# Lymphatus/caesium-clt

Hardware: AMD Instinct MI355X
Metric: megapixels/sec JPEG q=80 1920x1080 batch (higher is better)
Workload: dtype int32

## Files before the change

### caesium-clt_amd/csrc/batch.hpp

```cpp
#pragma once
#include <array>
#include <chrono>
#include <map>
#include <string>
#include <vector>

#include "../../include/caesium_hip.h"
#include "devmem.hpp"
#include "jpeg_host.hpp"
#include "kernels.h"
#include "webp_kernels.h"

namespace csh {

struct Item {
    int code = 0;
    std::string msg;
    JpegInfo in;
    JpegInfo out;
    int image = -1;
    size_t file_size = 0;
    std::vector<uint8_t> meta_out;
};

// ... 41 lines not shown
    uint32_t max_src_px = 0;
    uint64_t plane_bytes = 0, oplane_bytes = 0;
    uint32_t max_quads = 0;
    bool any_layout = false, any_layout_rgb = false;

    DevBuf<uint8_t> d_planes, d_oplanes, d_rgb;
    DevBuf<PlaneWork> d_pwork;
    DevBuf<ResizeWork> d_rwork;
    DevBuf<ResizeTap> d_rtaps;
    DevBuf<float> d_rweights, d_rtmp;
    DevBuf<int16_t> d_dct_raw;
};

struct Stage {
    uint32_t work0 = 0, nwork = 0, slot0 = 0, nslots = 0, ech0 = 0, nech = 0, table0 = 0, ntables = 0, plan0 = 0, nplans = 0, nzc0 = 0, nnzc = 0, ls0 = 0, nls = 0, ts0 = 0, nts = 0, rs0 = 0, nrs = 0, lr0 = 0, nlr = 0, rr0 = 0, nrr = 0;
    bool nz_build[2] = {true, true}, nz_filter[2] = {true, true};
};
struct SearchImg {
    int cand_work[64]; int ncand;
    int Al_luma = 0, Al_chroma = 0;
    uint64_t best_luma = 0, best_chroma = 0;
    int split_luma = 0, split_chroma = 0;
    bool luma_on = false, chroma_on = false;
};

struct EncodePlan {
    std::vector<EncScan> script;
    std::vector<ScanWork> swork;
    uint32_t nslots = 0, nlist_slots = 0, ntok_slots = 0;
    uint32_t nref_slots = 0;
    uint32_t last_run_refine = 0;
    uint32_t list_run = CSH_LIST_RUN;
    uint32_t nlist_runs = 0, nref_runs = 0;
    uint32_t last_run_list_runs = 0;
    uint64_t total_corr = 0;
    uint64_t total_units = 0, total_words = 0;
    uint32_t max_units = 0;
    int ntables = 0;
    std::vector<TokPlan> plans;
    std::vector<int> plan_comp, plan_image;
    std::vector<EChunk> echunks;
    uint64_t tok_cap = 0;
    uint32_t tok_scale = 1;
    std::vector<TokRegion> regions;
    std::vector<uint32_t> region_est;
    uint32_t hist_rows = 0;
    std::vector<NzList> nzlists;
    std::vector<NzSet> nzsets;
    std::vector<int> nzset_of;
    std::vector<uint32_t> nzset_built;
    std::vector<int> nzset_comp, nzset_image;
    std::vector<NzChunk> nzchunks;
    std::vector<NzChunk> nzchunks_fused;
    uint32_t n_fused = 0;
    uint32_t last_run_fused = 0;
    uint32_t n_ac_lists = 0;
    uint32_t last_run_ac_lists = 0;
    std::vector<uint8_t> nzset_ac_lists;
    std::vector<uint32_t> nz_est, nz_worst;
    uint32_t nz_nrec = 0;
    uint64_t nz_cap = 0;
    bool search = false;
    enum { ST_1 = 0, ST_1B = 1, ST_2 = 2, ST_2B = 3, ST_2C = 4, ST_N = 5 };
    Stage stage[ST_N];
    void stage_begin(Stage &sg) {
        sg.work0 = uint32_t(swork.size()); sg.slot0 = nslots; sg.ech0 = uint32_t(echunks.size()); sg.table0 = uint32_t(ntables); sg.plan0 = uint32_t(plans.size());
// ... 116 lines not shown
    KS_FF_COUNT, KS_SCAN_SEARCH, KS_LAYOUT, KS_SCAN_IMAGES, KS_EMIT, KS_SPARE0, KS_SPARE1, KS_SPARE2, KS_COUNT,
    KS_WEBP_YUV = KS_XFORM_DIRECT, KS_WEBP_ENCODE = KS_RESAMPLE_FDCT, KS_WEBP_ASSEMBLE = KS_FIX_DUMMY
};
struct KernelSlotRow { KernelSlot slot; const char *name; int phase; };
constexpr KernelSlotRow kKernelSlots[] = {
    {KS_MEMSET_COEF, "memset_coef", 0},        {KS_UNSTUFF, "unstuff", 0},                 {KS_DEC_SPEC, "k_dec_spec", 0},
    {KS_DEC_RELAX0, "k_dec_relax0", 0},        {KS_DEC_RELAX, "k_dec_relax1_4", 0},        {KS_DEC_WRITE, "k_dec_write", 0},
    {KS_DC_SCATTER, "k_dc_scatter", 0},        {KS_REFINE_CHAINS, "k_refine_chains", 0},   {KS_DECODE_PROG_SEQ, "k_decode_prog+seq", 0},
    {KS_IDCT_PLANE, "k_idct_plane", 1},        {KS_RESIZE, "resize", 1},                   {KS_XFORM_DIRECT, "k_xform_direct", 1},
    {KS_RESAMPLE_FDCT, "k_resample+k_plane_fdct", 1}, {KS_FIX_DUMMY, "k_fix_dummy", 1},    {KS_MEMSET_ENC, "memset_enc", 2},
    {KS_TRELLIS_STATS, "trellis_stats", 1},    {KS_TRELLIS_AC, "k_trellis_ac", 1},         {KS_TRELLIS_DC, "k_trellis_dc", 1},
    {KS_NZLIST, "k_nzlist", 2},                {KS_TOKENS, "k_tokens", 2},                 {KS_LIST_STATS, "k_list_stats", 2},
    {KS_AC_RUNS, "k_ac_runs", 2},              {KS_GEN_TABLES, "k_gen_tables", 3},         {KS_CHUNK_SIZES, "k_chunk_sizes", 4},
    {KS_SCAN_CHUNK_BITS, "scan_chunk_bits", 4}, {KS_SCAN_LAYOUT, "scan_layout", 4},        {KS_PACK, "k_pack", 5},
    {KS_LIST_PACK, "k_list_pack", 5},          {KS_FF_COUNT, "k_ff_count", 6},             {KS_SCAN_SEARCH, "scan_search_stage2", 7},
    {KS_LAYOUT, "k_layout", 6},                {KS_SCAN_IMAGES, "scan_images", 6},         {KS_EMIT, "k_emit", 6},
    {KS_SPARE0, "", 7},                        {KS_SPARE1, "", 7},                         {KS_SPARE2, "", 7}};
constexpr bool kernel_slots_in_order() {
    for (int i = 0; i < int(sizeof kKernelSlots / sizeof kKernelSlots[0]); i++) if (kKernelSlots[i].slot != i) return false;
    return true;
}
static_assert(sizeof kKernelSlots / sizeof kKernelSlots[0] == CSH_NKERNELS && int(KS_COUNT) == int(CSH_NKERNELS), "one row per csh_timing.kernel_ms slot");
static_assert(kernel_slots_in_order(), "row i of kKernelSlots describes slot i");

struct PlanSwitches {
    std::string profile;
    bool nz_once = true;
    bool tr_sort = true;
    int prog_par = -1;
    bool fused_420 = true;
    bool nz_fused = true;
    bool ref_list = true;
    uint32_t list_run = CSH_LIST_RUN;
    bool ac_tiles = false;
    static PlanSwitches read();
};

struct Laps {
    const bool trace;
    std::chrono::steady_clock::time_point at = std::chrono::steady_clock::now();
    std::string text;
    Laps();
    void lap(const char *what);
};

struct BatchPlanner {
    csh_batch *const b;
    const CByteArray *const inputs;
    const size_t count;
    const CCSParameters *const p;
    const csp_pixels *const px;
    const PlanSwitches sw;
    const bool progressive;
    uint16_t qout_nat[64];
    int script_base3 = 0, script_base1 = 0;
    std::vector<std::pair<std::vector<uint8_t>, int>> hset_keys;
    std::map<std::vector<uint16_t>, int> quant_index;
    uint64_t plane_off = 64, oplane_off = 0;

    BatchPlanner(csh_batch *b, const CByteArray *inputs, size_t count, const CCSParameters *p, const csp_pixels *px);
    void begin();
    void parse();
    int reserve_pinned();
    int plan_image(size_t n);
    int plan_search_stages();
    int plan_trellis();
// ... 35 lines not shown
```

### caesium-clt_amd/csrc/batch_plan.cpp

```cpp
#include <algorithm>
#include <atomic>
#include <cmath>
#include <thread>

#include "batch.hpp"
#include "resize_host.h"

namespace csh {

static void build_dev_huff(const HuffSpec &h, DevHuff &d) {
    memset(&d, 0, sizeof d);
    for (int l = 0; l < 18; l++) d.maxcode[l] = -1;
    if (!h.present) return;
    int code = 0, p = 0;
    for (int l = 1; l <= 16; l++) {
        if (h.bits[l]) {
            d.valptr[l] = p - code;
            for (int i = 0; i < h.bits[l]; i++, p++, code++)
                if (l <= 9) {
                    int base = code << (9 - l);
                    for (int k = 0; k < (1 << (9 - l)); k++) d.look[(base + k) & 511] = uint16_t((l << 8) | h.vals[p]);
                }
            d.maxcode[l] = code - 1;
        }
// ... 166 lines not shown
    b->enc.regions.resize(b->enc.region_est.size());
    if (b->test_pool_shift < 0) b->test_pool_shift = getenv("CSH_TEST_POOL_SHIFT") ? std::min(16, std::max(0, atoi(getenv("CSH_TEST_POOL_SHIFT")))) : 0;
    const int shift = b->test_pool_shift;
    uint64_t at = 0;
    for (size_t i = 0; i < b->enc.regions.size(); i++) {
        const uint64_t cap = std::min<uint64_t>(std::max<uint64_t>((uint64_t(b->enc.region_est[i]) * b->enc.tok_scale) >> shift, 64), 0xFFFFFFF0ull);
        b->enc.regions[i].base = at; b->enc.regions[i].cap = uint32_t(cap); b->enc.regions[i].pad = 0;
        at += (cap + 3) & ~uint64_t(3);
    }
    b->enc.tok_cap = at + 64;
    at = 0;
    for (size_t i = 0; i < b->enc.nzlists.size(); i++) {
        const uint64_t cap = std::min<uint64_t>(std::max<uint64_t>((uint64_t(b->enc.nz_est[i]) * b->enc.tok_scale) >> shift, 64), b->enc.nz_worst[i]);
        b->enc.nzlists[i].base = at; b->enc.nzlists[i].cap = uint32_t(cap);
        at += (cap + 3) & ~uint64_t(3);
    }
    b->enc.nz_cap = at + 64;
}

PlanSwitches PlanSwitches::read() {
    auto is = [](const char *name, const char *v) { const char *e = getenv(name); return e && !strcmp(e, v); };
    PlanSwitches s;
    const char *penv = getenv("CSH_PROFILE");
    s.profile = penv && *penv ? penv : "mozjpeg";
    s.nz_once = !is("CSH_NZ_ONCE", "0");
    s.tr_sort = !is("CSH_TR_SORT", "0");
    s.nz_fused = !is("CSH_NZ_FUSED", "0");
    s.ac_tiles = is("CSH_AC_TILES", "1");
    s.ref_list = is("CSH_REF_LIST", "1") || (s.ref_list && !is("CSH_REF_LIST", "0"));
    const char *pp = getenv("CSH_PROG_PAR");
    s.prog_par = pp && !strcmp(pp, "0") ? 0 : (pp && !strcmp(pp, "1") ? 1 : -1);
    s.fused_420 = !getenv("CSH_NO_FUSED_420");
    if (const char *lr = getenv("CSH_LIST_RUN")) { if (*lr) s.list_run = uint32_t(std::min(32, std::max(1, atoi(lr)))); }
    return s;
}

Laps::Laps() : trace(getenv("CSH_TRACE") != nullptr) {}
void Laps::lap(const char *what) {
    if (!trace) return;
    const auto now = std::chrono::steady_clock::now();
    char buf[64];
    snprintf(buf, sizeof buf, " %s %.1f", what, std::chrono::duration<double, std::milli>(now - at).count());
    text += buf; at = now;
}

BatchPlanner::BatchPlanner(csh_batch *b_, const CByteArray *inputs_, size_t count_, const CCSParameters *p_, const csp_pixels *px_)
    : b(b_), inputs(inputs_), count(count_), p(p_), px(px_), sw(PlanSwitches::read()), progressive(p_->jpeg_progressive) {}

void BatchPlanner::begin() {
    b->items.resize(count);
    quality_table(int(p->jpeg_quality), qout_nat);
    DevQuant qo; make_quant(qout_nat, qo);
    b->quants.push_back(qo);
    b->q_base = int(b->quants.size()) - 1;
    for (int q = 1; q <= 100; q++) { uint16_t tq[64]; quality_table(q, tq); DevQuant dq; make_quant(tq, dq); b->quants.push_back(dq); }
    b->progressive = progressive;
    b->enc.list_run = sw.list_run;

    add_script(b->enc.script, 3, true);
    add_script(b->enc.script, 1, true);
    add_script(b->enc.script, 3, false);
    add_script(b->enc.script, 1, false);
    script_base3 = progressive ? 0 : 16; script_base1 = progressive ? 10 : 17;
    const bool webp = b->webp, rgb_out = b->rgb_out;
    const std::string &profile = sw.profile;
    b->enc.search = progressive && !webp && !rgb_out && profile != "plain";
    const bool lossy_jpeg = !b->lossless && !webp && !rgb_out;
    b->tr.trellis = lossy_jpeg && (profile == "mozjpeg" || profile == "mozjpeg-trellis");
    b->tr.dering = lossy_jpeg && (profile == "mozjpeg" || profile == "mozjpeg-dering");
    b->tr.nz_once = b->tr.trellis && progressive && sw.nz_once && sw.tr_sort;
}

template <class Fill>
int BatchPlanner::enc_scan(const std::array<int, 5> &key, Fill fill) {
    auto f = b->enc.cand_script.find(key);
    if (f != b->enc.cand_script.end()) return f->second;
    EncScan e;
    memset(&e, 0, sizeof e);
    fill(e);
    b->enc.script.push_back(e);
    return b->enc.cand_script[key] = int(b->enc.script.size()) - 1;
}
int BatchPlanner::cand_index(int comp, int Ss, int Se, int Ah, int Al) {
    return enc_scan({comp, Ss, Se, Ah, Al}, [&](EncScan &e) {
        const int id = comp ? 1 : 0;
        e.ncomp = 1; e.comp[0] = comp; e.Ss = Ss; e.Se = Se; e.Ah = Ah; e.Al = Al;
        e.ntables = 1; e.dht_id[0] = 0x10 | id; e.sos_tdta[0] = id;
    });
}
int BatchPlanner::dc_scan_index(int ncomp) {
// ... 824 lines not shown
```

### caesium-clt_amd/csrc/batch_run.cpp

```cpp
#include <algorithm>

#include "batch.hpp"

namespace csh {
namespace {

class KernelMarks {
    hipEvent_t ev[CSH_NKERNELS + 1];
    int created = 0, next = 0;
    const hipStream_t st;

public:
    explicit KernelMarks(hipStream_t s) : st(s) {}
    KernelMarks(const KernelMarks &) = delete;
    KernelMarks &operator=(const KernelMarks &) = delete;
    ~KernelMarks() { for (int i = 0; i < created; i++) (void)hipEventDestroy(ev[i]); }
    int start() {
        for (; created <= CSH_NKERNELS; created++) CSH_CHECK(hipEventCreate(&ev[created]));
        CSH_CHECK(hipEventRecord(ev[0], st));
        return 0;
    }
    int claim(KernelSlot slot, hipEvent_t *e) {
        if (int(slot) != next || next >= CSH_NKERNELS) {
            csh_set_error("internal: timing mark '%s' out of order (slot %d is next)", slot < KS_COUNT ? kKernelSlots[slot].name : "?", next);
// ... 213 lines not shown
        }
        tc.ac_lists = fused ? 1u : 0u;
        tc.debug = getenv("CSH_TR_DEBUG") ? uint32_t(atoi(getenv("CSH_TR_DEBUG"))) : 0u;
    }

    int encode_begin() {
        fill_enc_ctx();
        launch_reset_works(st, b->enc.d_swork.p, c.nwork);
        if (!fused && (b->enc.d_nz_cursor.zero(st) || b->enc.d_nz_chunk_cnt.zero(st))) return -1;
        if (b->enc.d_symbits.zero(st) || b->enc.d_eobbits.zero(st) || (!eobrun_cleared && b->enc.d_eobrun.zero(st)) || b->enc.d_tables.zero(st) || b->enc.d_tok_cursor.zero(st) || b->enc.d_slot_eobh.zero(st) || b->enc.d_scan_pad.zero(st)) return -1;
#ifdef CSH_EMUL
        if (b->enc.d_raw.zero(st)) return -1;
#else
        if ((c.debug & 8192u) && b->enc.d_raw.zero(st)) return -1;
#endif
        MARK(KS_MEMSET_ENC);
        return 0;
    }

    void count_list_runs(const Stage &sg, bool gate) {
        for (uint32_t wi = sg.work0; (sg.nlr || sg.nrr) && wi < sg.work0 + sg.nwork; wi++) {
            const ScanWork &w = b->enc.swork[wi];
            if ((w.lr_base != 0xFFFFFFFFu || w.rr_base != 0xFFFFFFFFu) && (!gate || b->enc.work_active[wi])) b->enc.last_run_list_runs += ((w.nunits + 255u) / 256u + b->enc.list_run - 1u) / b->enc.list_run;
        }
    }

    void set_stage(const Stage &sg) {
        c.echunks = b->enc.d_echunks.p + sg.ech0; c.nechunks = sg.nech; c.slot0 = sg.slot0; c.nslots = sg.nslots;
        c.nzchunks = (fused ? b->enc.d_nzchunks_fused.p : b->enc.d_nzchunks.p) + sg.nzc0; c.nnzchunks = sg.nnzc;
        c.nz_build = sg.nz_build[fused ? 1 : 0]; c.nz_filter = sg.nz_filter[fused ? 1 : 0];
        c.list_slots = b->enc.d_list_slots.p + sg.ls0; c.nlist_slots = sg.nls; c.tok_slots = b->enc.d_tok_slots.p + sg.ts0; c.ntok_slots = sg.nts;
        c.ref_slots = b->enc.d_ref_slots.p + sg.rs0; c.nref_slots = sg.nrs;
        c.list_runs = b->enc.d_list_runs.p + sg.lr0; c.nlist_runs = sg.nlr; c.ref_runs = b->enc.d_ref_runs.p + sg.rr0; c.nref_runs = sg.nrr; c.list_run = b->enc.list_run;
    }

    int trellis() {
        const Stage &tg = b->tr.tstage;
        set_stage(tg);
        c.stats_only = 1;
        if (b->enc.d_long_cnt.zero(st)) return -1;
        c.nz_blk_cnt = b->tr.t_sort ? b->tr.d_tblk_cnt.p : nullptr;
        c.nz_blk_off = (b->tr.t_sort && b->tr.nz_once) ? b->tr.d_tblk_off.p : nullptr;
        launch_nzlist(st, c);
        c.nz_blk_cnt = nullptr; c.nz_blk_off = nullptr;
        if (b->tr.t_sort) {
            TrellisCtx ts;
            memset(&ts, 0, sizeof ts);
            ts.work = b->tr.d_twork.p; ts.nwork = int(b->tr.twork.size()); ts.blk_cnt = b->tr.d_tblk_cnt.p; ts.perm = b->tr.d_tperm.p;
            launch_trellis_sort(st, ts);
        }
        launch_tokens(st, c);
        launch_list_stats(st, c);
        count_list_runs(tg, false);
        launch_ac_runs(st, c);
        launch_gen_tables(st, b->enc.d_tables.p + tg.table0, int(tg.ntables));
        c.stats_only = 0;
        if (b->enc.d_nz_cursor.zero(st)) return -1;
        MARK(KS_TRELLIS_STATS);
        TrellisCtx tc;
        fill_trellis_ctx(tc);
        if (b->tr.d_tqueue.zero(st)) return -1;
        launch_trellis_ac(st, tc);
        MARK(KS_TRELLIS_AC);
        launch_trellis_dc(st, tc);
        launch_fix_dummy(st, b->d_imgs.p, nimg, b->max_dummy, b->d_coef.p);
        MARK(KS_TRELLIS_DC);
// ... 142 lines not shown
```

### caesium-clt_amd/csrc/k_entropy.hip

```cpp
#include "kernels.h"
#include "wave.h"

namespace csh {

#define CSH_PK_WORDS 1024

__device__ __forceinline__ static uint64_t band_mask(int Ss, int Se) { return (~0ull >> (63 - Se)) & (~0ull << Ss); }
__device__ __forceinline__ static int msb64(uint64_t v) { return 63 - __clzll(v); }
__device__ __forceinline__ static int bitlen32(unsigned v) { return 32 - __clz(v); }
__device__ __forceinline__ static int lane_id() { return int(threadIdx.x & 63); }

__device__ __forceinline__ static int unit_block(const CompGeom &g, uint32_t u) {
    int by = int(u) / g.real_bw, bx = int(u) - by * g.real_bw;
    return by * g.bw + bx;
}
__device__ __forceinline__ static bool get_bit(const uint64_t *w, uint32_t i) { return (w[i >> 6] >> (i & 63)) & 1; }

#ifndef CSH_EMUL
template <class Op>
__device__ __forceinline__ static uint32_t wave_scan_dpp(uint32_t v, Op op) {
    v = op(v, uint32_t(__builtin_amdgcn_update_dpp(0, int(v), 0x111, 0xf, 0xf, false)));
    v = op(v, uint32_t(__builtin_amdgcn_update_dpp(0, int(v), 0x112, 0xf, 0xf, false)));
    v = op(v, uint32_t(__builtin_amdgcn_update_dpp(0, int(v), 0x114, 0xf, 0xf, false)));
    v = op(v, uint32_t(__builtin_amdgcn_update_dpp(0, int(v), 0x118, 0xf, 0xf, false)));
// ... 421 lines not shown
                out.pos = 0;
                const uint64_t hi = pick_sig(pl, a.Al + 1), H = hi & band, N = lo & ~hi & band;
                if (c.debug & 8u) continue;
                emit_ac_refine(out, hist + slot * 257, uint32_t(tid), H, N, sgn, a.Ss, !((N >> a.Se) & 1), cnt[slot][tid] & 0xFFFFu);
                const uint32_t rawbits = uint32_t(__popcll(N) + __popcll(H));
                if (rawbits) atomicAdd(&s_raw[slot], rawbits);
            }
            continue;
        }
        if (c.debug & 32u) continue;
        if (ch.kind == 1) {
            const ScanWork &w = s_w;
            const EncScan &sc = s_sc;
            const SlotRec &r = c.slots[w.first_chunk + ch.j];
            for (uint32_t i = uint32_t(tid); i < uint32_t(sc.ntables) * 256u; i += 256) {
                const uint32_t v = hist[(i >> 8) * 257u + (i & 255u)];
                c.slot_hist[size_t(r.hist_row) * 256u + i] = uint16_t(v);
                if (v) atomicAdd(&c.tables[w.table_base + (i >> 8)].freq[i & 255u], v);
            }
            if (tid == 0) c.slot_raw[w.first_chunk + ch.j] = s_raw[0];
        } else {
            for (int slot = 0; slot < int(P.nslot); slot++) {
                const AcSlot &a = P.s[slot];
                const uint32_t cs = a.first_chunk + ch.j;
                const uint32_t v = hist[slot * 257 + tid];
                if (!(c.debug & 64u)) c.slot_hist[size_t(c.slots[cs].hist_row) * 256u + uint32_t(tid)] = uint16_t(v);
                if (v && !(c.debug & 128u)) atomicAdd(&c.tables[a.table_base].freq[tid], v);
                if (tid == 0) c.slot_raw[cs] = s_raw[slot];
            }
        }
    }
}

template <class Count>
__device__ static void eob_run_serial(const EncCtx &c, const ScanWork &w, const EncScan &sc, uint32_t u, uint32_t t, Count count) {
    uint16_t *er = c.eobrun + w.unit_base;
    if (sc.Ah == 0) {
        uint32_t L = t - u + 1, pos = u;
        while (L > 0) { uint32_t l = L < 0x7FFF ? L : 0x7FFF; er[pos] = uint16_t(l); count(l, pos); pos += l; L -= l; }
        return;
    }
    const uint8_t *tl = c.tail + w.unit_base;
    uint32_t cnt = 0, be = 0, s0 = u;
    auto step = [&](uint32_t j, uint32_t tail_bits) {
        cnt++; be += tail_bits;
        if (cnt == 0x7FFF || be > 937) { er[s0] = uint16_t(cnt); count(cnt, s0); cnt = 0; be = 0; s0 = j + 1; }
    };
    uint32_t j = u;
    while (j <= t && (reinterpret_cast<uintptr_t>(tl + j) & 7)) { step(j, tl[j]); j++; }
    for (; j + 7 <= t; j += 8) {
        const uint64_t v = *reinterpret_cast<const uint64_t *>(tl + j);
        CSH_UNROLL
        for (int i = 0; i < 8; i++) step(j + i, uint32_t(v >> (8 * i)) & 255u);
    }
    for (; j <= t; j++) step(j, tl[j]);
    if (cnt) { er[s0] = uint16_t(cnt); count(cnt, s0); }
}
__device__ static bool eob_run_end(const uint64_t *sym, uint32_t nunits, uint32_t u, uint32_t max_words, uint32_t &t) {
    t = nunits - 1;
    uint32_t i = u + 1;
    const uint32_t nwords = (nunits + 63) >> 6;
    for (uint32_t n = 0; i < nunits; n++) {
        if (n == max_words) return false;
        uint32_t wi = i >> 6;
        uint64_t bits = sym[wi] & (~0ull << (i & 63));
        if (bits) { uint32_t p = (wi << 6) + uint32_t(__ffsll((unsigned long long)bits) - 1); if (p < nunits) t = p - 1; return true; }
        i = (wi + 1) << 6;
        if (wi + 1 >= nwords) break;
    }
    return true;
}
#define CSH_LONG_RUN_WORDS 8
__global__ void __launch_bounds__(256) k_ac_runs(EncCtx c) {
    const int lane = lane_id();
    const uint32_t cs = c.slot0 + blockIdx.x * 4u + (threadIdx.x >> 6);
    if (cs >= c.slot0 + c.nslots) return;
    const SlotRec r = c.slots[cs];
    if (!(r.flags & 1u)) return;
    if (c.work_active && !c.work_active[r.work]) return;
    const uint32_t nunits = r.nunits_work;
    uint32_t *freq = c.tables[r.table_base].freq;
    const uint64_t *sym = c.sym_bits + r.word_base, *eob = c.eob_bits + r.word_base;
    uint32_t mine = 0;
    (void)mine; (void)lane;
    CSH_UNROLL
    for (int i = 0; i < 4; i++) {
        const uint32_t u = r.j * 256u + uint32_t(i) * 64u + uint32_t(lane);
        int my_nb = -1;
        if (u < nunits) {
            const uint32_t w0 = u >> 6, nwords = (nunits + 63) >> 6;
            const int bit = int(u & 63);
            const uint64_t s0 = sym[w0], e0 = eob[w0];
            const uint64_t s1 = w0 + 1 < nwords ? sym[w0 + 1] : ~0ull;
            const bool prev_eob = u == 0 ? false : (bit ? ((e0 >> (bit - 1)) & 1) != 0 : ((eob[w0 - 1] >> 63) & 1) != 0);
            const bool start = ((e0 >> bit) & 1) && (((s0 >> bit) & 1) || !prev_eob);
            if (start) {
                const uint64_t a0 = bit == 63 ? 0ull : (s0 & (~0ull << (bit + 1)));
                uint32_t next = 0xFFFFFFFFu;
                if (a0) next = (w0 << 6) + uint32_t(__ffsll((unsigned long long)a0) - 1);
                else if (s1) next = ((w0 + 1) << 6) + uint32_t(__ffsll((unsigned long long)s1) - 1);
                if (next != 0xFFFFFFFFu && next > nunits) next = nunits;
                const uint32_t len = next == 0xFFFFFFFFu ? 0xFFFFFFFFu : next - u;
                if (len <= 14u || (len < 0x7FFFu && r.Ah == 0)) {
                    c.eobrun[r.unit_base + u] = uint16_t(len);
                    my_nb = bitlen32(len) - 1;
                } else {
                    ScanWork w; w.unit_base = r.unit_base; w.word_base = r.word_base; w.nunits = nunits; w.first_chunk = r.first_chunk; w.table_base = r.table_base;
                    EncScan sc; sc.Ss = r.Ss; sc.Se = r.Se; sc.Ah = r.Ah; sc.Al = r.Al;
                    uint32_t t;
                    if (eob_run_end(sym, nunits, u, CSH_LONG_RUN_WORDS, t))
                        eob_run_serial(c, w, sc, u, t, [&](uint32_t run, uint32_t owner) {
                            const int nb = bitlen32(run) - 1;
                            atomicAdd(&freq[nb << 4], 1u); atomicAdd(&c.slot_eobh[size_t(r.first_chunk + (owner >> 8)) * 16u + uint32_t(nb)], 1u);
                        });
                    else { uint32_t e = atomicAdd(c.long_cnt, 1u); c.long_runs[2 * e] = r.work; c.long_runs[2 * e + 1] = u; }
                }
            }
        }
#ifdef CSH_EMUL
        if (my_nb >= 0) { atomicAdd(&freq[my_nb << 4], 1u); atomicAdd(&c.slot_eobh[cs * 16u + uint32_t(my_nb)], 1u); }
#else
        CSH_UNROLL
        for (int nb = 0; nb < 4; nb++) {
            const uint64_t m = __ballot(my_nb == nb);
            if (lane == nb) mine += uint32_t(__popcll(m));
        }
        if (__ballot(my_nb >= 4)) {
            for (int nb = 4; nb < 15; nb++) {
                const uint64_t m = __ballot(my_nb == nb);
                if (lane == nb) mine += uint32_t(__popcll(m));
            }
        }
#endif
    }
#ifndef CSH_EMUL
    if (mine && lane < 15) { atomicAdd(&freq[lane << 4], mine); atomicAdd(&c.slot_eobh[cs * 16u + uint32_t(lane)], mine); }
#endif
}
__global__ void __launch_bounds__(64) k_ac_runs_long(EncCtx c) {
    const uint32_t n = *c.long_cnt;
    for (uint32_t e = blockIdx.x; e < n; e += gridDim.x) {
        const ScanWork w = c.work[c.long_runs[2 * e]];
        const EncScan &sc = c.script[w.scan];
        const uint32_t u = c.long_runs[2 * e + 1];
        const uint64_t *sym = c.sym_bits + w.word_base;
        uint32_t *freq = c.tables[w.table_base].freq;
        auto count = [&](uint32_t run, uint32_t owner) {
            const int nb = bitlen32(run) - 1;
            atomicAdd(&freq[nb << 4], 1u); atomicAdd(&c.slot_eobh[size_t(w.first_chunk + (owner >> 8)) * 16u + uint32_t(nb)], 1u);
        };
#ifdef CSH_EMUL
        uint32_t t;
        eob_run_end(sym, w.nunits, u, 0xFFFFFFFFu, t);
        eob_run_serial(c, w, sc, u, t, count);
#else
        const uint32_t lane = threadIdx.x, nwords = (w.nunits + 63) >> 6;
        uint32_t t = w.nunits - 1;
        for (uint32_t w0 = (u + 1) >> 6; w0 < nwords; w0 += 64) {
            uint64_t bits = w0 + lane < nwords ? sym[w0 + lane] : 0ull;
            if (w0 + lane == ((u + 1) >> 6)) bits &= ~0ull << ((u + 1) & 63);
            const uint64_t hit = __ballot(bits != 0);
            if (hit) {
                const int l0 = __ffsll((unsigned long long)hit) - 1;
                const uint32_t lo = uint32_t(__shfl(int(uint32_t(bits)), l0, 64)), hi = uint32_t(__shfl(int(uint32_t(bits >> 32)), l0, 64));
                const uint64_t b = (uint64_t(hi) << 32) | lo;
                const uint32_t p = ((w0 + uint32_t(l0)) << 6) + uint32_t(__ffsll((unsigned long long)b) - 1);
                if (p < w.nunits) t = p - 1;
                break;
            }
        }
// ... 398 lines not shown
    CSH_WAVE_FENCE();
    PackState S; S.buf = buf; S.out = out; S.pos = pos; S.ww = ww; S.first_flush = first_flush;
    if (!in_lds) pack_segments<3>(c, x, S, cs, pad, lane);
    else if (!(r.flags & 1u)) pack_segments<3>(c, xl, S, cs, pad, lane);
    else if (r.flags & 2u) pack_segments<2>(c, xl, S, cs, pad, lane);
    else pack_segments<1>(c, xl, S, cs, pad, lane);
    pos = S.pos; ww = S.ww; first_flush = S.first_flush;
    CSH_WAVE_FENCE();
    const uint32_t last = uint32_t((pos + 31) >> 5) - ww;
    for (uint32_t q = uint32_t(lane); q < last; q += 64) {
        const uint32_t v = buf[q];
        if ((first_flush && q == 0) || q == last - 1) { if (v) atomicOr(out + ww + q, v); } else out[ww + q] = v;
    }
#endif
}

__global__ void __launch_bounds__(256) k_zero_edges(EncCtx c) {
    const uint32_t cs = c.slot0 + blockIdx.x * 256u + threadIdx.x;
    if (cs >= c.slot0 + c.nslots) return;
    const SlotRec r = c.slots[cs];
    const ScanWork &w = c.work[r.work];
    if (w.no_room || (c.work_active && !c.work_active[r.work])) return;
    const uint64_t scan0 = c.chunk_off[r.first_chunk];
    const uint64_t bit0 = w.raw_off * 8 + (c.chunk_off[cs] - scan0);
    const uint64_t nbits = c.chunk_bits[cs];
    c.raw[bit0 >> 5] = 0;
    const uint64_t lo = nbits ? (bit0 + nbits - 1) >> 5 : bit0 >> 5, hi = (bit0 + nbits + (r.j == r.nch - 1 ? 8 : 0)) >> 5;
    for (uint64_t wi = lo; wi <= hi; wi++) c.raw[wi] = 0;
}
void launch_zero_edges(hipStream_t st, const EncCtx &c) { if (c.nslots) CSH_LAUNCH(k_zero_edges, dim3((c.nslots + 255) / 256), dim3(256), st, c); }
void launch_tokens(hipStream_t st, const EncCtx &c) { if (c.nechunks) CSH_LAUNCH_PHASED(k_tokens, 6, dim3(c.nechunks), dim3(256), st, c); }
void launch_ac_runs(hipStream_t st, const EncCtx &c) {
    if (!c.nslots) return;
    CSH_LAUNCH(k_ac_runs, dim3((c.nslots + 3) / 4), dim3(256), st, c);
#ifdef CSH_EMUL
    CSH_LAUNCH(k_ac_runs_long, dim3(64), dim3(1), st, c);
#else
    CSH_LAUNCH(k_ac_runs_long, dim3(4096), dim3(64), st, c);
#endif
}
void launch_chunk_sizes(hipStream_t st, const EncCtx &c) { if (c.nslots) CSH_LAUNCH(k_chunk_sizes, dim3((c.nslots + 3) / 4), dim3(256), st, c); }
void launch_pack(hipStream_t st, const EncCtx &c) { if (c.ntok_slots) CSH_LAUNCH(k_pack, dim3((c.ntok_slots + 3) / 4), dim3(256), st, c); }

}
```

### caesium-clt_amd/csrc/kernels.h

```cpp
#pragma once
#include "gpu_rt.h"
#include "types.h"

namespace csh {

__host__ __device__ static inline int coef_off(int k) { return (k >> 3) * CSH_OCT_STRIDE + (k & 7); }
__host__ __device__ static inline size_t coef_index(uint32_t tile_base, int b, int k) {
    return (size_t(tile_base) + size_t(b >> 6)) * CSH_TILE_I16 + size_t((b & 63) * CSH_BLK_STRIDE) + size_t(coef_off(k));
}

#define CSH_RAW_OCT 8
__host__ __device__ static inline size_t raw_index(uint32_t tile_base, int b) { return size_t(tile_base) * CSH_TILE_I16 + size_t(b) * 64; }

__device__ __forceinline__ static int csh_plane_at(const uint8_t *p, int pitch, int cw, int ch, int y, int x) {
    y = y < 0 ? 0 : (y > ch - 1 ? ch - 1 : y);
    x = x < 0 ? 0 : (x > cw - 1 ? cw - 1 : x);
    return p[size_t(y) * pitch + x];
}
__device__ __forceinline__ static int csh_upsample_at(const uint8_t *p, int pitch, int cw, int ch, UpDesc u, int r, int xx) {
    switch (u.cls) {
    case CSH_UP_COPY: return csh_plane_at(p, pitch, cw, ch, r, xx);
    case CSH_UP_H2V1: {
        const int cx = xx >> 1, nb = (xx & 1) ? cx + 1 : cx - 1;
        return (3 * csh_plane_at(p, pitch, cw, ch, r, cx) + csh_plane_at(p, pitch, cw, ch, r, nb) + ((xx & 1) ? 2 : 1)) >> 2;
// ... 95 lines not shown
    uint32_t *slot_raw;
    uint32_t *slot_eobh;
    uint32_t *chunk_bits;
    const uint64_t *chunk_off;
    DevEncTable *tables;
    uint32_t *raw;
    uint64_t raw_words;
    uint32_t *status;
    uint32_t *overflow;
    uint32_t debug;
    uint32_t stats_only;
    const uint8_t *work_active;
    const NzList *nzlists;
    const NzSet *nzsets;
    const NzChunk *nzchunks;
    uint32_t nnzchunks;
    uint32_t *nz_pool;
    uint32_t *nz_cursor;
    uint32_t *nz_chunk_off;
    uint32_t *nz_chunk_cnt;
    uint8_t *nz_blk_cnt;
    uint16_t *nz_blk_off;
    const uint32_t *list_slots;
    uint32_t nlist_slots;
    const uint32_t *tok_slots;
    uint32_t ntok_slots;
    const uint32_t *ref_slots;
    uint32_t nref_slots;
    const uint32_t *list_runs;
    uint32_t nlist_runs;
    const uint32_t *ref_runs;
    uint32_t nref_runs;
    uint32_t list_run;
    uint32_t nz_build, nz_filter;
};
enum : uint32_t { TK_SYM = 0u, TK_RAW = 1u, TK_ACF = 2u, TK_REF = 3u, TK_EOB = 4u };
void launch_tokens(hipStream_t st, const EncCtx &c);
void launch_ac_runs(hipStream_t st, const EncCtx &c);
void launch_gen_tables(hipStream_t st, DevEncTable *tables, int ntables);
void launch_chunk_sizes(hipStream_t st, const EncCtx &c);
void launch_zero_edges(hipStream_t st, const EncCtx &c);
void launch_pack(hipStream_t st, const EncCtx &c);
void launch_nzlist(hipStream_t st, const EncCtx &c);
void launch_list_stats(hipStream_t st, const EncCtx &c);
void launch_list_refine(hipStream_t st, const EncCtx &c);
void launch_list_pack(hipStream_t st, const EncCtx &c);
void launch_nz_to_tiles(hipStream_t st, const NzSet *nzsets, const NzList *nzlists, const uint32_t *nz_pool, const uint32_t *nz_chunk_off, const uint32_t *nz_chunk_cnt,
                        uint32_t set, uint32_t nchunks, int16_t *coef);
void launch_reset_works(hipStream_t st, ScanWork *work, int nwork);

#ifndef CSH_LIST_RUN
#define CSH_LIST_RUN 8
#endif
#ifndef CSH_TR_WG
#define CSH_TR_WG 256
#endif
#ifndef CSH_TR_RUN
#define CSH_TR_RUN 8
#endif
struct TrellisCtx {
    const ImgDesc *imgs;
    const DevQuant *quant;
    const TrellisWork *work;
    int nwork;
    const TrellisRun *runs;
    uint32_t nruns;
// ... 66 lines not shown
```

### caesium-clt_amd/csrc/pipeline.cpp

```cpp
#include <algorithm>
#include <atomic>
#include <cmath>
#include <cstdarg>
#include <memory>
#include <thread>

#include "batch.hpp"
#include "../../include/vp8_tables.h"
#include "resize_host.h"

static thread_local char g_err[512];
void csh_set_error(const char *fmt, ...) {
    va_list ap;
    va_start(ap, fmt);
    vsnprintf(g_err, sizeof g_err, fmt, ap);
    va_end(ap);
}
extern "C" const char *csh_last_error(void) { return g_err; }

#ifdef CSH_EMUL
thread_local dim3 threadIdx, blockIdx, blockDim, gridDim;
int csh_emul_reverse = 0;
thread_local int csh_emul_phase = 0;
extern "C" void csh_emul_set_reverse(int r) { csh_emul_reverse = r; }
namespace csh { extern int csh_emul_jacobi; }
extern "C" void csh_emul_set_jacobi(int j) { csh::csh_emul_jacobi = j; }
#endif

using namespace csh;

static float sincf_(float t) { float a = t * 3.14159265358979323846f; return t == 0.0f ? 1.0f : sinf(a) / a; }
static float lanczos3f(float x) { return fabsf(x) < 3.0f ? sincf_(x) * sincf_(x / 3.0f) : 0.0f; }
void csh_lanczos_axis(int in_size, int out_size, bool identity, std::vector<ResizeTap> &taps, std::vector<float> &weights) {
    for (int o = 0; o < out_size; o++) {
        ResizeTap t;
        t.woff = uint32_t(weights.size());
        if (identity) { t.left = o; t.n = 1; weights.push_back(1.0f); taps.push_back(t); continue; }
        float ratio = float(in_size) / float(out_size);
        float sratio = ratio < 1.0f ? 1.0f : ratio;
        float support = 3.0f * sratio;
        float center = (float(o) + 0.5f) * ratio;
        long left = long(floorf(center - support)); if (left < 0) left = 0; if (left > in_size - 1) left = in_size - 1;
        long right = long(ceilf(center + support)); if (right < left + 1) right = left + 1; if (right > in_size) right = in_size;
        center = center - 0.5f;
        float sum = 0.0f;
        for (long i = left; i < right; i++) { float w = lanczos3f((float(i) - center) / sratio); weights.push_back(w); sum += w; }
        for (size_t i = t.woff; i < weights.size(); i++) weights[i] /= sum;
        t.left = int(left); t.n = int(right - left);
        taps.push_back(t);
    }
}
void csh_compute_dimensions(int ow, int oh, int dw, int dh, int &nw, int &nh) {
    if (dw > 0 && dh > 0) { nw = dw; nh = dh; }
    else {
        float ratio = float(ow) / float(oh);
        if (dw > 0) { nw = dw; nh = int(roundf(float(dw) / ratio)); }
        else { nh = dh; nw = int(roundf(float(dh) * ratio)); }
    }
    if (nw < 1) nw = 1;
// ... 291 lines not shown
```

Before: 44850.

## Add word-parallel AC EOB-run kernel processing 16 slots per wave

Adds k_ac_runs_words, a new default kernel for the AC EOB-run pass. Each wave loads the sym/eob bitmask words for 16 slots (four words per slot, one per lane group), then walks them with one lane per bit, counting run-length histograms via ballots. It accumulates frequency atomics per work item before flushing, which cuts global atomic traffic and gives each thread more work than the per-slot kernel. The old per-slot kernel stays reachable with CSH_AC_RUNS=slot, and emulator-only path counters are added. The cost is a serial loop over slots inside each wave and lower parallelism when there are few slots.

```diff
diff --git a/caesium-clt_amd/csrc/batch.hpp b/caesium-clt_amd/csrc/batch.hpp
--- a/caesium-clt_amd/csrc/batch.hpp
+++ b/caesium-clt_amd/csrc/batch.hpp
@@ -97,6 +97,7 @@
     uint32_t last_run_refine = 0;
     uint32_t list_run = CSH_LIST_RUN;
     uint32_t nlist_runs = 0, nref_runs = 0;
+    bool ac_runs_slot = false;
     uint32_t last_run_list_runs = 0;
     uint64_t total_corr = 0;
     uint64_t total_units = 0, total_words = 0;
@@ -279,6 +280,7 @@
     bool nz_fused = true;
     bool ref_list = true;
     uint32_t list_run = CSH_LIST_RUN;
+    bool ac_runs_slot = false;
     bool ac_tiles = false;
     static PlanSwitches read();
 };
diff --git a/caesium-clt_amd/csrc/batch_plan.cpp b/caesium-clt_amd/csrc/batch_plan.cpp
--- a/caesium-clt_amd/csrc/batch_plan.cpp
+++ b/caesium-clt_amd/csrc/batch_plan.cpp
@@ -222,6 +222,7 @@
     s.prog_par = pp && !strcmp(pp, "0") ? 0 : (pp && !strcmp(pp, "1") ? 1 : -1);
     s.fused_420 = !getenv("CSH_NO_FUSED_420");
     if (const char *lr = getenv("CSH_LIST_RUN")) { if (*lr) s.list_run = uint32_t(std::min(32, std::max(1, atoi(lr)))); }
+    s.ac_runs_slot = is("CSH_AC_RUNS", "slot");
     return s;
 }
 
@@ -246,6 +247,7 @@
     for (int q = 1; q <= 100; q++) { uint16_t tq[64]; quality_table(q, tq); DevQuant dq; make_quant(tq, dq); b->quants.push_back(dq); }
     b->progressive = progressive;
     b->enc.list_run = sw.list_run;
+    b->enc.ac_runs_slot = sw.ac_runs_slot;
 
     add_script(b->enc.script, 3, true);
     add_script(b->enc.script, 1, true);
diff --git a/caesium-clt_amd/csrc/batch_run.cpp b/caesium-clt_amd/csrc/batch_run.cpp
--- a/caesium-clt_amd/csrc/batch_run.cpp
+++ b/caesium-clt_amd/csrc/batch_run.cpp
@@ -269,6 +269,7 @@
         c.list_slots = b->enc.d_list_slots.p + sg.ls0; c.nlist_slots = sg.nls; c.tok_slots = b->enc.d_tok_slots.p + sg.ts0; c.ntok_slots = sg.nts;
         c.ref_slots = b->enc.d_ref_slots.p + sg.rs0; c.nref_slots = sg.nrs;
         c.list_runs = b->enc.d_list_runs.p + sg.lr0; c.nlist_runs = sg.nlr; c.ref_runs = b->enc.d_ref_runs.p + sg.rr0; c.nref_runs = sg.nrr; c.list_run = b->enc.list_run;
+        c.ac_runs_slot = b->enc.ac_runs_slot ? 1u : 0u;
     }
 
     int trellis() {
diff --git a/caesium-clt_amd/csrc/k_entropy.hip b/caesium-clt_amd/csrc/k_entropy.hip
--- a/caesium-clt_amd/csrc/k_entropy.hip
+++ b/caesium-clt_amd/csrc/k_entropy.hip
@@ -477,6 +477,12 @@
     }
 }
 
+#ifdef CSH_EMUL
+uint32_t csh_emul_ac_paths[8];
+#define CSH_ACR_PATH(i) ((void)csh_emul_ac_paths[i]++)
+#else
+#define CSH_ACR_PATH(i) ((void)0)
+#endif
 template <class Count>
 __device__ static void eob_run_serial(const EncCtx &c, const ScanWork &w, const EncScan &sc, uint32_t u, uint32_t t, Count count) {
     uint16_t *er = c.eobrun + w.unit_base;
@@ -489,7 +495,7 @@
     uint32_t cnt = 0, be = 0, s0 = u;
     auto step = [&](uint32_t j, uint32_t tail_bits) {
         cnt++; be += tail_bits;
-        if (cnt == 0x7FFF || be > 937) { er[s0] = uint16_t(cnt); count(cnt, s0); cnt = 0; be = 0; s0 = j + 1; }
+        if (cnt == 0x7FFF || be > 937) { CSH_ACR_PATH(cnt == 0x7FFF ? 7 : 3); er[s0] = uint16_t(cnt); count(cnt, s0); cnt = 0; be = 0; s0 = j + 1; }
     };
     uint32_t j = u;
     while (j <= t && (reinterpret_cast<uintptr_t>(tl + j) & 7)) { step(j, tl[j]); j++; }
@@ -549,16 +555,18 @@
                 if (len <= 14u || (len < 0x7FFFu && r.Ah == 0)) {
                     c.eobrun[r.unit_base + u] = uint16_t(len);
                     my_nb = bitlen32(len) - 1;
+                    CSH_ACR_PATH(0);
                 } else {
                     ScanWork w; w.unit_base = r.unit_base; w.word_base = r.word_base; w.nunits = nunits; w.first_chunk = r.first_chunk; w.table_base = r.table_base;
                     EncScan sc; sc.Ss = r.Ss; sc.Se = r.Se; sc.Ah = r.Ah; sc.Al = r.Al;
                     uint32_t t;
-                    if (eob_run_end(sym, nunits, u, CSH_LONG_RUN_WORDS, t))
+                    if (eob_run_end(sym, nunits, u, CSH_LONG_RUN_WORDS, t)) {
+                        CSH_ACR_PATH(1); if (r.Ah) CSH_ACR_PATH(2);
                         eob_run_serial(c, w, sc, u, t, [&](uint32_t run, uint32_t owner) {
                             const int nb = bitlen32(run) - 1;
                             atomicAdd(&freq[nb << 4], 1u); atomicAdd(&c.slot_eobh[size_t(r.first_chunk + (owner >> 8)) * 16u + uint32_t(nb)], 1u);
                         });
-                    else { uint32_t e = atomicAdd(c.long_cnt, 1u); c.long_runs[2 * e] = r.work; c.long_runs[2 * e + 1] = u; }
+                    } else { CSH_ACR_PATH(4); uint32_t e = atomicAdd(c.long_cnt, 1u); c.long_runs[2 * e] = r.work; c.long_runs[2 * e + 1] = u; }
                 }
             }
         }
@@ -581,6 +589,97 @@
 #ifndef CSH_EMUL
     if (mine && lane < 15) { atomicAdd(&freq[lane << 4], mine); atomicAdd(&c.slot_eobh[cs * 16u + uint32_t(lane)], mine); }
 #endif
+}
+#define CSH_ACR_SLOTS 16u
+__global__ void __launch_bounds__(256) k_ac_runs_words(EncCtx c) {
+    const uint32_t cs0 = c.slot0 + (blockIdx.x * 4u + uni(uint32_t(threadIdx.x) / CSP_WAVE_THREADS)) * CSH_ACR_SLOTS, cs_end = c.slot0 + c.nslots;
+    if (cs0 >= cs_end) return;
+    LV<uint32_t> ok, s_lo, s_hi, e_lo, e_hi, n_lo, n_hi, prev, word, unit_base, nunits, scan4, table, first, word_base, work;
+    LFOR(l) {
+        const uint32_t cs = cs0 + (uint32_t(l) >> 2);
+        ok[l] = 0u; s_lo[l] = s_hi[l] = e_lo[l] = e_hi[l] = n_lo[l] = n_hi[l] = prev[l] = 0u;
+        word[l] = unit_base[l] = nunits[l] = scan4[l] = table[l] = first[l] = word_base[l] = work[l] = 0u;
+        if (cs < cs_end) {
+            const SlotRec &r = c.slots[cs];
+            const uint32_t w = 4u * r.j + (uint32_t(l) & 3u), nwords = (r.nunits_work + 63u) >> 6;
+            if ((r.flags & 1u) && w < nwords && !(c.work_active && !c.work_active[r.work])) {
+                const uint64_t *sym = c.sym_bits + r.word_base, *eob = c.eob_bits + r.word_base;
+                const uint64_t s0 = sym[w], e0 = eob[w];
+                const uint64_t s1 = w + 1 < nwords ? sym[w + 1] : ~0ull;
+                ok[l] = 1u; s_lo[l] = uint32_t(s0); s_hi[l] = uint32_t(s0 >> 32); e_lo[l] = uint32_t(e0); e_hi[l] = uint32_t(e0 >> 32); n_lo[l] = uint32_t(s1); n_hi[l] = uint32_t(s1 >> 32);
+                prev[l] = w ? uint32_t(eob[w - 1] >> 63) : 0u;
+                word[l] = w; unit_base[l] = r.unit_base; nunits[l] = r.nunits_work; table[l] = r.table_base; first[l] = r.first_chunk; word_base[l] = r.word_base; work[l] = r.work;
+                scan4[l] = uint32_t(r.Ss) | (uint32_t(r.Se) << 8) | (uint32_t(r.Ah) << 16) | (uint32_t(r.Al) << 24);
+            }
+        }
+    }
+    const uint64_t okm = lballot([&](int l) { return ok[l] != 0u; });
+    if (!okm) return;
+    if ((okm & 1u) && lget(word, 0u) != 0u) CSH_ACR_PATH(6);
+    LV<uint32_t> mine, facc;
+    LFOR(l) { mine[l] = 0u; facc[l] = 0u; }
+    uint32_t acc_work = 0xFFFFFFFFu, acc_table = 0u;
+    auto flush_freq = [&]() { LFOR(l) if (facc[l] && l < 15) { atomicAdd(&c.tables[acc_table].freq[l << 4], facc[l]); facc[l] = 0u; } };
+    for (uint32_t q = 0; q < CSH_ACR_SLOTS; q++) {
+        if (!((okm >> (4u * q)) & 15u)) continue;
+        for (uint32_t i = 4u * q; i < 4u * q + 4u; i++) {
+            if (!((okm >> i) & 1u)) continue;
+            const uint64_t s0 = (uint64_t(lget(s_hi, i)) << 32) | lget(s_lo, i), e0 = (uint64_t(lget(e_hi, i)) << 32) | lget(e_lo, i);
+            const uint32_t wk = lget(work, i), table_base = lget(table, i);
+            if (wk != acc_work) { if (acc_work != 0xFFFFFFFFu) CSH_ACR_PATH(5); flush_freq(); acc_work = wk; acc_table = table_base; }
+            if (!e0) continue;
+            const uint64_t s1 = (uint64_t(lget(n_hi, i)) << 32) | lget(n_lo, i);
+            const uint32_t prev_top = lget(prev, i), w0 = lget(word, i), ubase = lget(unit_base, i), nun = lget(nunits, i), sc4 = lget(scan4, i), first_chunk = lget(first, i), wbase = lget(word_base, i);
+            const uint32_t Ah = (sc4 >> 16) & 255u;
+            uint32_t *freq = c.tables[table_base].freq;
+            LV<int> my_nb;
+            LFOR(b) {
+                my_nb[b] = -1;
+                const uint32_t u = (w0 << 6) + uint32_t(b);
+                if (u < nun) {
+                    const int bit = b;
+                    const bool prev_eob = bit ? ((e0 >> (bit - 1)) & 1) != 0 : prev_top != 0u;
+                    const bool start = ((e0 >> bit) & 1) && (((s0 >> bit) & 1) || !prev_eob);
+                    if (start) {
+                        const uint64_t a0 = bit == 63 ? 0ull : (s0 & (~0ull << (bit + 1)));
+                        uint32_t next = 0xFFFFFFFFu;
+                        if (a0) next = (w0 << 6) + uint32_t(__ffsll((unsigned long long)a0) - 1);
+                        else if (s1) next = ((w0 + 1) << 6) + uint32_t(__ffsll((unsigned long long)s1) - 1);
+                        if (next != 0xFFFFFFFFu && next > nun) next = nun;
+                        const uint32_t len = next == 0xFFFFFFFFu ? 0xFFFFFFFFu : next - u;
+                        if (len <= 14u || (len < 0x7FFFu && Ah == 0)) {
+                            c.eobrun[ubase + u] = uint16_t(len);
+                            my_nb[b] = bitlen32(len) - 1;
+                            CSH_ACR_PATH(0);
+                        } else {
+                            ScanWork w; w.unit_base = ubase; w.word_base = wbase; w.nunits = nun; w.first_chunk = first_chunk; w.table_base = table_base;
+                            EncScan sc; sc.Ss = uint8_t(sc4); sc.Se = uint8_t(sc4 >> 8); sc.Ah = uint8_t(sc4 >> 16); sc.Al = uint8_t(sc4 >> 24);
+                            uint32_t t;
+                            if (eob_run_end(c.sym_bits + wbase, nun, u, CSH_LONG_RUN_WORDS, t)) {
+                                CSH_ACR_PATH(1); if (Ah) CSH_ACR_PATH(2);
+                                eob_run_serial(c, w, sc, u, t, [&](uint32_t run, uint32_t owner) {
+                                    const int nb = bitlen32(run) - 1;
+                                    atomicAdd(&freq[nb << 4], 1u); atomicAdd(&c.slot_eobh[size_t(first_chunk + (owner >> 8)) * 16u + uint32_t(nb)], 1u);
+                                });
+                            } else { CSH_ACR_PATH(4); uint32_t e = atomicAdd(c.long_cnt, 1u); c.long_runs[2 * e] = wk; c.long_runs[2 * e + 1] = u; }
+                        }
+                    }
+                }
+            }
+            for (int nb = 0; nb < 4; nb++) {
+                const uint32_t n = popc64(lballot([&](int b) { return my_nb[b] == nb; }));
+                LFOR(l) if (l == nb) mine[l] += n;
+            }
+            if (lballot([&](int b) { return my_nb[b] >= 4; })) {
+                for (int nb = 4; nb < 15; nb++) {
+                    const uint32_t n = popc64(lballot([&](int b) { return my_nb[b] == nb; }));
+                    LFOR(l) if (l == nb) mine[l] += n;
+                }
+            }
+        }
+        LFOR(l) if (mine[l] && l < 15) { atomicAdd(&c.slot_eobh[size_t(cs0 + q) * 16u + uint32_t(l)], mine[l]); facc[l] += mine[l]; mine[l] = 0u; }
+    }
+    flush_freq();
 }
 __global__ void __launch_bounds__(64) k_ac_runs_long(EncCtx c) {
     const uint32_t n = *c.long_cnt;
@@ -1045,7 +1144,8 @@
 void launch_tokens(hipStream_t st, const EncCtx &c) { if (c.nechunks) CSH_LAUNCH_PHASED(k_tokens, 6, dim3(c.nechunks), dim3(256), st, c); }
 void launch_ac_runs(hipStream_t st, const EncCtx &c) {
     if (!c.nslots) return;
-    CSH_LAUNCH(k_ac_runs, dim3((c.nslots + 3) / 4), dim3(256), st, c);
+    if (c.ac_runs_slot) CSH_LAUNCH(k_ac_runs, dim3((c.nslots + 3) / 4), dim3(256), st, c);
+    else CSH_LAUNCH(k_ac_runs_words, dim3((c.nslots + 4u * CSH_ACR_SLOTS - 1u) / (4u * CSH_ACR_SLOTS)), dim3(4 * CSP_WAVE_THREADS), st, c);
 #ifdef CSH_EMUL
     CSH_LAUNCH(k_ac_runs_long, dim3(64), dim3(1), st, c);
 #else
diff --git a/caesium-clt_amd/csrc/kernels.h b/caesium-clt_amd/csrc/kernels.h
--- a/caesium-clt_amd/csrc/kernels.h
+++ b/caesium-clt_amd/csrc/kernels.h
@@ -151,6 +151,7 @@
     const uint32_t *ref_runs;
     uint32_t nref_runs;
     uint32_t list_run;
+    uint32_t ac_runs_slot;
     uint32_t nz_build, nz_filter;
 };
 enum : uint32_t { TK_SYM = 0u, TK_RAW = 1u, TK_ACF = 2u, TK_REF = 3u, TK_EOB = 4u };
diff --git a/caesium-clt_amd/csrc/pipeline.cpp b/caesium-clt_amd/csrc/pipeline.cpp
--- a/caesium-clt_amd/csrc/pipeline.cpp
+++ b/caesium-clt_amd/csrc/pipeline.cpp
@@ -25,6 +25,8 @@
 extern "C" void csh_emul_set_reverse(int r) { csh_emul_reverse = r; }
 namespace csh { extern int csh_emul_jacobi; }
 extern "C" void csh_emul_set_jacobi(int j) { csh::csh_emul_jacobi = j; }
+namespace csh { extern uint32_t csh_emul_ac_paths[8]; }
+extern "C" void csh_emul_ac_paths(uint32_t *out) { for (int i = 0; i < 8; i++) { out[i] = csh::csh_emul_ac_paths[i]; csh::csh_emul_ac_paths[i] = 0u; } }
 #endif
 
 using namespace csh;
```

Result: faster. 45420, median of 6 (+1.3%).
